# Dunni3/keypoint-diffusion

Measured on AMD Instinct MI355X. Metric: denoising steps/sec, higher is better.
Workload: dtype f32; 1 GPU; egnn_all_atom dynamics (6 EGNN layers, hidden 256, update_kp_feat; fixed receptor encoder), batch of 64 synthetic 300-atom pockets / 25-atom ligands per GPU, T=500, seeded random-init weights, every step taken from the t=T ligand state; batch_per_gpu=64, n_rec=300, n_lig=25, parallelism=dp1

## Files before the change

keypoint-diffusion_amd/csrc/egnn.hip:

```cpp
#include <string.h>

#include <map>
#include <set>
#include <string>
#include <vector>

#include "egnn_kernels.h"
#include "egnn_wide.h"
#include "mfma_core.h"

using namespace kpd;

namespace {

struct LayerW {
    float *wp_e[4], *wx_e[4], *b_e[4], *wr_e[4], *watt[4];
    float *wp_c[4], *wx_c[4], *b_c[4], *wr_c[4], *w3[4];
    void *wh_e[4], *wh_c[4];
    void *chh_p[2][NSLOT];
    void *wh_a[2], *wh_b[2], *wh_2[2];
    float *wp_p[2][NSLOT], *wx_p[2][NSLOT], *b_p[2][NSLOT];
    float *ch_p[2][NSLOT], *wcol_p[2][NSLOT];
    float *wp_a[2], *wx_a[2], *wp_b[2], *wx_b[2], *b0[2], *wp_2[2], *wx_2[2], *b2[2], *ln_w[2], *ln_b[2];
};
// ... 57 lines not shown
    int cap_B = 0, cap_lig = 0, cap_kp = 0, cap_kk = 0, cap_ll = 0, cap_kl = 0, cap_maxlig = 0, cap_maxkp = 0;
    int tile_cap = 0, tiles_et_cap[4] = {0, 0, 0, 0};
    float *h[2], *x[2], *P[2];
    float *hn_main[4], *hn_cont[4], *xn_main[4], *xn_cont[4];
    int *bidx[2];
    float *z[2];
    int *meta, *ll_deg, *ll_off, *kl_off, *kl_pg;
    kpd_lig_graph lg;
    int kp_table = 1;
    int tab_rows = 0;
    bool last_table = false;
    int *rowmap = nullptr, *kp_ok = nullptr;
    float *tab_in = nullptr;
    int *tab_bidx = nullptr;
    float *hT = nullptr, *PT = nullptr;
    EgnnWide *wide = nullptr;
};

static kpd_status build_weight_arena(kpd_egnn *m) {
    const kpd_egnn_config &c = m->cfg;
    m->warena.poison_at = 2;
    m->L.assign(c.n_layers, LayerW());
    return carve(m->warena, ARENA_TAIL, [&](Carve &A) {
        for (int i = 0; i < c.n_layers; ++i) {
            LayerW &w = m->L[i];
            const std::string pre = "egnn.conv_layers." + std::to_string(i) + ".";
            for (int et = 0; et < m->n_et; ++et) {
                A(w.wp_e[et], WP_FLOATS); A(w.wx_e[et], HS); A(w.b_e[et], HS); A(w.wr_e[et], HS); A(w.watt[et], HS);
                A(w.wp_c[et], WP_FLOATS); A(w.wx_c[et], HS); A(w.b_c[et], HS); A(w.wr_c[et], HS); A(w.w3[et], HS);
                A.as<unsigned short>(w.wh_e[et], WH_HALVES); A.as<unsigned short>(w.wh_c[et], WH_HALVES);
// ... 393 lines not shown
        }
        for (int et = 0; et < 4; ++et) {
            W.rows(m->hn_main[et], n[kDstNt[et]], HS, HW);
            W.rows(m->hn_cont[et], tiles[et], HS, HW);
            W(m->xn_main[et], (size_t)n[kDstNt[et]] * 4);
            W(m->xn_cont[et], (size_t)tiles[et] * 4);
        }
        carve_lig_graph(W, m->meta, m->ll_deg, m->ll_off, m->kl_off, m->kl_pg, g, max_B, max_n_lig, max_n_kp);
        if (tab_rows > 0) {
            W(m->rowmap, max_n_kp);
            W(m->kp_ok, 1);
            W(m->tab_in, (size_t)tab_rows * rec_nf);
            W(m->tab_bidx, tab_rows);
            W(m->hT, (size_t)(tab_rows + TM) * HS);
            W.rows(m->PT, (size_t)(tab_rows + TM) * NSLOT, HS, HW);
        }
    }));
    m->tab_rows = tab_rows;
    m->last_table = false;
    if (tab_rows > 0) {
        std::vector<float> in((size_t)tab_rows * rec_nf, 0.0f);
        std::vector<int> gi(tab_rows);
        for (int r = 0; r < tab_rows; ++r) {
            in[(size_t)r * rec_nf + r % rec_nf] = 1.0f;
            gi[r] = r / rec_nf;
        }
        KPD_HIP(hipMemcpy(m->tab_in, in.data(), in.size() * 4, hipMemcpyHostToDevice));
        KPD_HIP(hipMemcpy(m->tab_bidx, gi.data(), gi.size() * 4, hipMemcpyHostToDevice));
    }
    for (int et = 0; et < 4; ++et) m->tiles_et_cap[et] = tiles[et];
// ... 26 lines not shown
    if (kp_tab)
        KPD_TRY(launch_node_graph_index(bt->kp_ptr, bt->B, bt->n_kp, m->bidx[NT_KP], st, nullptr, bt->kp_h, c.rec_nf, m->rowmap, m->kp_ok));
    else
        KPD_TRY(launch_node_graph_index(bt->kp_ptr, bt->B, bt->n_kp, m->bidx[NT_KP], st));
    const float *x_cur[2] = {bt->lig_x, bt->kp_x};
    KPD_TRY(launch_lig_graph(bt, c.ll_cutoff, c.ll_k, c.kl_cutoff, c.kl_k, &m->lg, m->ll_deg, m->ll_off, m->kl_off, m->kl_pg, st));
    const int tr = TM;
    const int active = c.update_kp_feat ? 0xF : 0x3;
    const bool prune = c.update_kp_feat && m->prune_last;
    const int active_last = prune ? 0x3 : active;
    KPD_TRY(launch_egnn_meta(m->lg.counts, bt->n_kk, active, active_last, bt->lig_ptr, bt->kp_ptr, m->lg.ll_per_graph,
                             bt->kk_rowptr, bt->B, m->kl_off, c.message_norm, c.update_kp_feat, m->meta, m->z[NT_LIG],
                             m->z[NT_KP], st, tr));
    KPD_TRY(launch_embed(bt->lig_h, bt->n_lig, c.atom_nf, m->le_W0, m->le_b0, 64, m->le_W1t, m->le_b1, t_dev,
                         m->bidx[NT_LIG], m->h[NT_LIG], 0, st));
    KPD_TRY(launch_embed(bt->kp_h, bt->n_kp, c.rec_nf, m->re_W0, m->re_b0, 2 * c.rec_nf, m->re_W1t, m->re_b1, t_dev,
                         m->bidx[NT_KP], m->h[NT_KP], m->rec_identity ? 1 : 0, st));
    if (kp_tab) {
        KPD_REQUIRE(n_tab <= m->tab_rows, KPD_ERR_CAPACITY, "internal: %d class rows, table of %d", n_tab, m->tab_rows);
        KPD_TRY(launch_embed(m->tab_in, n_tab, c.rec_nf, m->re_W0, m->re_b0, 2 * c.rec_nf, m->re_W1t, m->re_b1, t_dev, m->tab_bidx,
                             m->hT, 0, st));
    }

    const int e_kl_cap = bt->n_kp * (c.kl_k > 0 ? c.kl_k : std::min(bt->max_lig, 100));
    const int E_cap[4] = {std::max<int>((long)bt->n_lig * std::min(bt->max_lig - 1, c.ll_k > 0 ? c.ll_k : 200), 1), e_kl_cap, e_kl_cap,
                          bt->n_kk};
    int tile_cap = 0, tile_cap_last = 0;
    for (int et = 0; et < m->n_et; ++et) {
        tile_cap += cdiv(E_cap[et], tr);
        if ((active_last >> et) & 1) tile_cap_last += cdiv(E_cap[et], tr);
    }

    const int n[2] = {bt->n_lig, bt->n_kp};
    const int *esrc[4] = {m->lg.ll_src, m->lg.kl_src, m->lg.lk_src, bt->kk_src};
    const int *edst[4] = {m->lg.ll_dst, m->lg.kl_dst, m->lg.lk_dst, bt->kk_dst};
    const int *rowptr[4] = {m->lg.ll_rowptr, m->lg.kl_rowptr, m->lg.lk_rowptr, bt->kk_rowptr};
    const int n_layers = m->debug_layers >= 0 ? std::min(m->debug_layers, c.n_layers) : c.n_layers;

    auto slot_mask = [&](int etmask, int nt) {
        int mk = 0;
        for (int et = 0; et < 4; ++et)
            if ((etmask >> et) & 1) {
                if (kSrcNt[et] == nt) mk |= 3 << kSrcSlot[et];
                if (kDstNt[et] == nt) mk |= 3 << kDstSlot[et];
            }
        return mk;
    };
    auto layer_etmask = [&](int li) { return li == n_layers - 1 ? active_last : active; };
    for (int li = 0; li < n_layers; ++li) {
        const LayerW &L = m->L[li];
        {
            {
// ... 8 lines not shown
                        if (L.wp_p[nt][s] && ((mk >> s) & 1)) {
                            pa.wp[k] = L.wp_p[nt][s]; pa.wx[k] = L.wx_p[nt][s]; pa.bias[k] = L.b_p[nt][s]; pa.slot[k] = s;
                            pa.chain[k] = L.ch_p[nt][s]; pa.wcol[k] = L.wcol_p[nt][s]; pa.chain_h[k] = L.chh_p[nt][s];
                            ++k;
                        }
                    pp.n_slots[nt] = k;
                }
                pp.tiles0 = cdiv(n[0], TM);
                pp.gemm_mode = m->gemm_mode;
                if (kp_tab && li == 0) {
                    ProjPair pk = pp;
                    pk.n_slots[NT_LIG] = 0;
                    pk.skip_if = m->kp_ok;
                    ProjArgs &pa = pp.nt[NT_KP];
                    pa.h = m->hT; pa.n = n_tab; pa.P = m->PT;
                    KPD_TRY(launch_proj_chain(pp, st));
                    KPD_TRY(launch_proj_chain(pk, st));
                } else {
                    KPD_TRY(launch_proj_chain(pp, st));
                }
            }
        }
        EdgeArgs ea;
        memset(&ea, 0, sizeof(ea));
        const bool last = li == n_layers - 1;
        ea.meta = last ? m->meta + 16 : m->meta;
        ea.x[0] = x_cur[0]; ea.x[1] = x_cur[1]; ea.P[0] = m->P[0]; ea.P[1] = m->P[1];
        ea.use_tanh = c.use_tanh; ea.coords_range = c.coords_range;
        ea.tile_rows = tr;
        ea.gemm_mode = tr == TM ? m->gemm_mode : 0;
        for (int et = 0; et < 4; ++et) {
            ea.src[et] = esrc[et]; ea.dst[et] = edst[et];
            ea.src_nt[et] = kSrcNt[et]; ea.dst_nt[et] = kDstNt[et]; ea.src_slot[et] = kSrcSlot[et]; ea.dst_slot[et] = kDstSlot[et];
            ea.wr_e[et] = L.wr_e[et]; ea.wr_c[et] = L.wr_c[et];
// ... 28 lines not shown
            na.ln_inv_n = 1.0f / (float)(c.hidden_nf + 1); na.ln_pad = (float)(HID - c.hidden_nf);
            na.wh_a = L.wh_a[nt]; na.wh_b = L.wh_b[nt]; na.wh_2 = L.wh_2[nt];
            na.norm = c.norm;
            na.tile_shift = 6;
        };
        {
            NodeLayerPair lp;
            memset(&lp, 0, sizeof(lp));
            for (int nt = 0; nt < 2; ++nt) {
                NodeLayerArgs &na = lp.nt[nt];
                na.u.n = n[nt]; na.u.h = m->h[nt];
                if (nt < m->n_upd && !(nt == NT_KP && last && prune)) {
                    fill_update(na.u, nt);
                    na.u.x_in = x_cur[nt] == m->x[nt] ? nullptr : x_cur[nt];
                    na.do_update = 1;
                }
                if (!na.do_update && !na.do_proj) na.u.n = 0;
            }
            lp.tiles0 = cdiv(lp.nt[0].u.n, TN);
            lp.gemm_mode = m->gemm_mode;
            KPD_TRY(launch_node_layer(lp, st));
            for (int nt = 0; nt < 2; ++nt)
                if (lp.nt[nt].do_update) x_cur[nt] = m->x[nt];
        }
    }
    if (x_cur[NT_LIG] != m->x[NT_LIG]) KPD_HIP(hipMemcpyAsync(m->x[NT_LIG], bt->lig_x, (size_t)bt->n_lig * 12, hipMemcpyDeviceToDevice, st));
    if (x_cur[NT_KP] != m->x[NT_KP]) KPD_HIP(hipMemcpyAsync(m->x[NT_KP], bt->kp_x, (size_t)bt->n_kp * 12, hipMemcpyDeviceToDevice, st));
    KPD_TRY(launch_decode(m->h[NT_LIG], m->x[NT_LIG], bt->lig_x, bt->n_lig, c.atom_nf, 2 * c.atom_nf, m->de_W0, m->de_b0,
                          m->de_W1, m->de_b1, eps_h, eps_x, st));
    return KPD_OK;
}

extern "C" kpd_status kpd_egnn_debug_state(kpd_egnn *m, const char *what, float *out, int64_t n_floats, void *stream) {
    KPD_REQUIRE(m && what && out, KPD_ERR_INVALID, "null argument");
    hipStream_t st = static_cast<hipStream_t>(stream);
    if (m->wide) return wide_debug_state(m->wide, what, out, n_floats, st);
    const std::string w(what);
    const float *src = nullptr;
    if (w == "h_lig") src = m->h[0];
    else if (w == "h_kp") src = m->h[1];
// ... 5 lines not shown
             w[3] >= '0' && w[3] < '4') {
        const int et = w[3] - '0';
        src = w[0] == 'x' ? (w[2] == 'm' ? m->xn_main[et] : m->xn_cont[et]) : (w[2] == 'm' ? m->hn_main[et] : m->hn_cont[et]);
    }
    else if (w == "kp_table_ok") {
        KPD_REQUIRE(n_floats == 1, KPD_ERR_INVALID, "kp_table_ok is one value");
        if (!m->last_table) {
            KPD_HIP(hipMemsetAsync(out, 0, 4, st));
            return KPD_OK;
        }
        src = reinterpret_cast<const float *>(m->kp_ok);
    } else if (w.rfind("kp_table=", 0) == 0) {
        m->kp_table = atoi(w.c_str() + 9);
        return KPD_OK;
    }
    else if (w.rfind("layers=", 0) == 0) {
        m->debug_layers = atoi(w.c_str() + 7);
        return KPD_OK;
    } else if (w.rfind("prune=", 0) == 0) {
        m->prune_last = atoi(w.c_str() + 6);
        return KPD_OK;
    } else if (w.rfind("gemm=", 0) == 0) {
        const std::string v = w.substr(5);
        KPD_REQUIRE(v == "f32" || v == "f16x2", KPD_ERR_INVALID, "gemm mode must be f32 or f16x2");
        KPD_REQUIRE(v == "f32" || !m->f32_only, KPD_ERR_INVALID,
                    "gemm=f16x2: atom_nf = %d / rec_nf = %d (hidden_nf = %d) run the exact fp32 path only; the f16x2 mode covers atom_nf <= 32 "
                    "with rec_nf <= 128 or 256, or the identity keypoint encoder at hidden_nf 256", m->cfg.atom_nf, m->cfg.rec_nf, m->cfg.hidden_nf);
        KPD_REQUIRE(v == "f32" || !m->committed || m->f16_ok, KPD_ERR_WEIGHTS, "%s", F16_RANGE_ERROR);
        m->gemm_mode = v == "f16x2" ? 1 : 0;
        return KPD_OK;
// ... 67 lines not shown
```

keypoint-diffusion_amd/csrc/egnn_chain.hip:

```cpp
#include <algorithm>
#include <cstdlib>

#include "chain_core.h"
#include "egnn_kernels.h"

namespace kpd {

namespace {

constexpr int ENT = 16;
constexpr int ECH4 = ENT * 64;

__device__ __forceinline__ float reduce_q(float v) {
    v += __shfl_xor(v, 16);
    v += __shfl_xor(v, 32);
    return v;
}

}

struct ProjWs {
    ProjPair p;
    int blocks0;
    int bpc[2];
    int tpb;
};

constexpr int WS_TILE = 128;
constexpr int WS_W4 = 16 * 8 * 64;
constexpr int WS_LDS_BYTES = WS_W4 * 16 + (128 + 128 + HS) * 4;

__global__ __launch_bounds__(512, 1) void k_proj_ws(ProjWs qa) {
    extern __shared__ __attribute__((aligned(16))) float smem[];
    v4f *W = reinterpret_cast<v4f *>(smem);
    float *s_wcol = smem + WS_W4 * 4, *s_bias = s_wcol + 128, *s_wrow = s_bias + 128;
    const int tid = threadIdx.x, wave = tid >> 6, lane = tid & 63;
    if (qa.p.skip_if && *qa.p.skip_if) return;
    const int which = (int)blockIdx.x >= qa.blocks0 ? 1 : 0;
    const ProjArgs &a = qa.p.nt[which];
    const int local = blockIdx.x - (which ? qa.blocks0 : 0);
    const int combo = local / qa.bpc[which], chunk = local - combo * qa.bpc[which];
    const int s = combo >> 1, hf = combo & 1;
    const int tiles = (a.n + WS_TILE - 1) / WS_TILE;
    const int t0 = chunk * qa.tpb, t1 = min(tiles, t0 + qa.tpb);
    if (t0 >= t1) return;
    {
        const v4f *src = reinterpret_cast<const v4f *>(a.chain[s]);
#pragma unroll
        for (int j = 0; j < WS_W4 / 512; ++j) {
            const int i = tid + 512 * j, ks = i >> 9, rem = i & 511;
            W[i] = src[(size_t)ks * ECH4 + 8 * hf * 64 + rem];
        }
        const float *bias = a.bias[s];
        if (tid < 128) {
            s_wcol[tid] = a.wcol[s][128 * hf + tid];
            s_bias[tid] = bias ? bias[128 * hf + tid] : 0.0f;
        }
        for (int i = tid; i < HS; i += 512) s_wrow[i] = i <= 256 ? a.wx[s][i] : 0.0f;
    }
    __syncthreads();
    const int el = lane & 15, q = lane >> 4;
    const float bias256 = a.bias[s] ? a.bias[s][256] : 0.0f;
    auto load_x = [&](int t, v4f (&x)[ENT], float &x256) {
        const int row = min(t * WS_TILE + 16 * wave + el, a.n - 1);
        const float *hrow = a.h + (size_t)row * HS;
#pragma unroll
        for (int nt = 0; nt < ENT; ++nt) x[nt] = *reinterpret_cast<const v4f *>(hrow + 16 * nt + 4 * q);
        x256 = hrow[256];
    };
    auto store_tile = [&](const v4f (&acc)[8], int row, float out256) {
        if (row >= 0 && row < a.n) {
            float *orow = a.P + ((size_t)row * NSLOT + a.slot[s]) * HS + 128 * hf;
#pragma unroll
            for (int m = 0; m < 8; ++m) *reinterpret_cast<v4f *>(orow + 16 * m + 4 * q) = acc[m];
            if (hf == 0 && q == 0) orow[256] = out256;
        }
    };
    v4f x[ENT], xn[ENT], accp[8];
    float h256, h256n, out256p = 0.0f;
    int rowp = -1;
#pragma unroll
    for (int m = 0; m < 8; ++m) accp[m] = zero4();
    load_x(t0, xn, h256n);
#pragma unroll 1
    for (int t = t0; t < t1; ++t) {
#pragma unroll
        for (int nt = 0; nt < ENT; ++nt)
#pragma unroll
            for (int r = 0; r < 4; ++r) asm volatile("v_mov_b32 %0, %1" : "=v"(x[nt][r]) : "v"(xn[nt][r]));
        asm volatile("v_mov_b32 %0, %1" : "=v"(h256) : "v"(h256n));
        __builtin_amdgcn_sched_barrier(0);
        store_tile(accp, rowp, out256p);
        if (t + 1 < t1) load_x(t + 1, xn, h256n);
        v4f acc[8];
#pragma unroll
        for (int m = 0; m < 8; ++m)
            acc[m] = h256 * *reinterpret_cast<const v4f *>(s_wcol + 16 * m + 4 * q) + *reinterpret_cast<const v4f *>(s_bias + 16 * m + 4 * q);
        float part = 0.0f;
        if (hf == 0) {
#pragma unroll
            for (int nt = 0; nt < ENT; ++nt) {
                const v4f wv = *reinterpret_cast<const v4f *>(s_wrow + 16 * nt + 4 * q);
                part += x[nt][0] * wv[0] + x[nt][1] * wv[1] + x[nt][2] * wv[2] + x[nt][3] * wv[3];
            }
        }
        const v4f *wp = W + lane;
        v4f w[2][4];
#pragma unroll
// ... 1 lines not shown
#pragma unroll
        for (int b = 0; b < 32; ++b) {
            if (b + 1 < 32) {
#pragma unroll
                for (int m = 0; m < 4; ++m) w[(b + 1) & 1][m] = wp[(4 * (b + 1) + m) * 64];
            }
            __builtin_amdgcn_sched_barrier(0);
            const v4f xin = x[b >> 1];
            const int g = b & 1;
#pragma unroll
            for (int r = 0; r < 4; ++r)
#pragma unroll
                for (int m = 0; m < 4; ++m) acc[4 * g + m] = mfma16(w[b & 1][m][r], xin[r], acc[4 * g + m]);
            __builtin_amdgcn_sched_barrier(0);
        }
        const int row = t * WS_TILE + 16 * wave + el;
        const float out256 = hf == 0 ? reduce_q(part) + bias256 + h256 * s_wrow[256] : 0.0f;
#pragma unroll
        for (int m = 0; m < 8; ++m) accp[m] = acc[m];
        rowp = row;
        out256p = out256;
    }
    store_tile(accp, rowp, out256p);
}

__global__ __launch_bounds__(512, 1) void k_proj_ws_h(ProjWs qa) {
    extern __shared__ __attribute__((aligned(16))) float smem[];
    f32x4 *W = reinterpret_cast<f32x4 *>(smem);
    float *s_wcol = smem + WS_W4 * 4, *s_bias = s_wcol + 128, *s_wrow = s_bias + 128;
    const int tid = threadIdx.x, wave = tid >> 6, lane = tid & 63;
    const int which = (int)blockIdx.x >= qa.blocks0 ? 1 : 0;
// ... 93 lines not shown
            acc[m0] = __builtin_amdgcn_mfma_f32_16x16x32_f16(as_h8(wb[1]), as_h8(xh[kb]), acc[m0], 0, 0, 0);
            acc[m0 + 1] = __builtin_amdgcn_mfma_f32_16x16x32_f16(as_h8(wb[3]), as_h8(xh[kb]), acc[m0 + 1], 0, 0, 0);
            acc[m0] = __builtin_amdgcn_mfma_f32_16x16x32_f16(as_h8(wb[0]), as_h8(xl[kb]), acc[m0], 0, 0, 0);
            acc[m0 + 1] = __builtin_amdgcn_mfma_f32_16x16x32_f16(as_h8(wb[2]), as_h8(xl[kb]), acc[m0 + 1], 0, 0, 0);
            acc[m0] = __builtin_amdgcn_mfma_f32_16x16x32_f16(as_h8(wb[0]), as_h8(xh[kb]), acc[m0], 0, 0, 0);
            acc[m0 + 1] = __builtin_amdgcn_mfma_f32_16x16x32_f16(as_h8(wb[2]), as_h8(xh[kb]), acc[m0 + 1], 0, 0, 0);
            __builtin_amdgcn_sched_barrier(0);
        }
#pragma unroll
        for (int m = 0; m < 8; ++m) accp[m] = H_UNSCALE * acc[m];
        rowp = row;
    }
    store_tile(accp, rowp);
}

kpd_status launch_proj_chain(const ProjPair &p, hipStream_t st) {
    const int slots = std::max(p.n_slots[0], p.n_slots[1]);
    if (poison_level() >= 1) KPD_TRY(poison_lds(st));
    if (slots == 0) return KPD_OK;
    for (int nt = 0; nt < 2; ++nt)
        for (int s = 0; s < p.n_slots[nt]; ++s)
            KPD_REQUIRE(p.nt[nt].chain[s] && p.nt[nt].wcol[s], KPD_ERR_STATE, "projection slot %d not packed", s);
    KPD_TRY(ensure_dynamic_lds(reinterpret_cast<const void *>(k_proj_ws), WS_LDS_BYTES));
    const int target = cu_count();
    ProjWs q;
    q.p = p;
    int units = 0, tl[2];
    for (int nt = 0; nt < 2; ++nt) {
        tl[nt] = p.n_slots[nt] ? cdiv(p.nt[nt].n, WS_TILE) : 0;
        units += 2 * p.n_slots[nt] * tl[nt];
    }
    if (units == 0) return KPD_OK;
    int blocks[2];
    for (q.tpb = std::max(1, cdiv(units, target));; ++q.tpb) {
        for (int nt = 0; nt < 2; ++nt) {
            q.bpc[nt] = std::max(1, cdiv(tl[nt], q.tpb));
            blocks[nt] = tl[nt] ? 2 * p.n_slots[nt] * q.bpc[nt] : 0;
        }
        if (blocks[0] + blocks[1] <= target || q.tpb >= std::max(tl[0], tl[1])) break;
    }
    q.blocks0 = blocks[0];
    if (p.gemm_mode == 1) {
        KPD_REQUIRE(!p.skip_if, KPD_ERR_INVALID, "projection launch: skip_if is served by the exact mode only");
        for (int nt = 0; nt < 2; ++nt)
            for (int s = 0; s < p.n_slots[nt]; ++s)
                KPD_REQUIRE(p.nt[nt].chain_h[s], KPD_ERR_STATE, "projection slot %d has no f16 planes (f16x2 mode)", s);
        KPD_TRY(ensure_dynamic_lds(reinterpret_cast<const void *>(k_proj_ws_h), WS_LDS_BYTES));
        hipLaunchKernelGGL(k_proj_ws_h, dim3(blocks[0] + blocks[1]), dim3(512), WS_LDS_BYTES, st, q);
        KPD_LAUNCH_CHECK();
        return KPD_OK;
    }
    hipLaunchKernelGGL(k_proj_ws, dim3(blocks[0] + blocks[1]), dim3(512), WS_LDS_BYTES, st, q);
    KPD_LAUNCH_CHECK();
    return KPD_OK;
}

}
```

keypoint-diffusion_amd/csrc/egnn_kernels.h:

```cpp
#pragma once
#include "engine.h"

namespace kpd {

constexpr int NSLOT = 8;
constexpr int ATT_BIAS_AT = 260;
constexpr int BIAS_K = 260;
constexpr int ET_LL = 0, ET_KL = 1, ET_LK = 2, ET_KK = 3;
constexpr int NT_LIG = 0, NT_KP = 1;

constexpr int EDGE_LDS_BYTES = TM * SA * 4 + (TM * 2 + TM + 3 * TM + TM + 3 * TM + 4 * HS + 8 + TM) * 4;
constexpr int EDGE_H_LDS_BYTES = 64 * 280 * 2 * 2 + (TM * 2 + TM + 3 * TM + TM + 3 * TM + 2 * HS + 8) * 4 + 2 * 2 * 272 * 2;

struct ProjArgs {
    const float *h;
    int n;
    float *P;
    const float *wp[NSLOT];
    const float *wx[NSLOT];
    const float *bias[NSLOT];
    int slot[NSLOT];
    const float *chain[NSLOT];
    const float *wcol[NSLOT];
    const void *chain_h[NSLOT];
// ... 86 lines not shown
    float *x;
    const float *x_in;
    const int *bidx;
    const float *z;
    int n_in;
    const int *rowptr[2];
    const float *hn_main[2], *hn_cont[2];
    const float *xn_main[2], *xn_cont[2];
    const float *wp_a, *wx_a, *wp_b, *wx_b, *b0;
    const float *wp_2, *wx_2, *b2;
    const void *wh_a, *wh_b, *wh_2;
    const float *ln_w, *ln_b;
    int norm;
    float ln_inv_n, ln_pad;
    int tile_shift;
};

struct NodeLayerArgs {
    NodeArgs u;
    int do_update, do_proj;
    float *P;
    int n_slots;
    const float *wp[NSLOT], *wx[NSLOT], *bias[NSLOT];
    int slot[NSLOT];
};

struct NodeLayerPair {
    NodeLayerArgs nt[2];
    int tiles0;
    int gemm_mode;
};

constexpr int TN = 32;
constexpr int NODE_LAYER_LDS_BYTES = TN * SA * 4 + 3 * TN * 4 + 3 * HS * 4;
constexpr int NODE_H_TILE_FLOATS = 2 * TN * 280 / 2;
constexpr int NODE_H_LDS_BYTES = NODE_H_TILE_FLOATS * 4 + 3 * TN * 4;


kpd_status egnn_kernels_init();
kpd_status launch_node_graph_index(const int *ptr, int B, int n, int *bidx, hipStream_t st, int *set_ok = nullptr,
                                   const float *kp_h = nullptr, int fin = 0, int *rowmap = nullptr, int *ok = nullptr);
kpd_status launch_egnn_meta(const int *counts, int e_kk, int active_mask, int active_last, const int *lig_ptr, const int *kp_ptr,
                            const int *ll_per_graph, const int *kk_rowptr, int B, const int *kl_off, float message_norm,
                            int update_kp, int *meta, float *z_lig, float *z_kp, hipStream_t st, int tile_rows = TM);
kpd_status launch_embed(const float *in, int n, int fin, const float *W0, const float *b0, int hid, const float *W1t,
                        const float *b1, const float *t, const int *bidx, float *out, int identity, hipStream_t st);
kpd_status launch_decode(const float *h, const float *x, const float *x0, int n, int atom_nf, int hid, const float *W0,
                         const float *b0, const float *W1, const float *b1, float *eps_h, float *eps_x, hipStream_t st);
kpd_status launch_egnn_edge(const EdgeArgs &a, int tile_cap, hipStream_t st);
kpd_status launch_egnn_edge_train(const EdgeTrainArgs &a, int tile_cap, hipStream_t st);
struct EdgePiecesSumArgs {
    const float *hn_main[4], *hn_cont[4], *xn_main[4], *xn_cont[4];
    const int *rowptr[4];
    int live[4], dst_nt[4];
    const float *zinv[2];
    int n[2];
    float *hn[2], *xn[2];
};
kpd_status launch_edge_pieces_sum(const EdgePiecesSumArgs &a, hipStream_t st);
kpd_status launch_edge_train_pack(const EdgePackTab &t, hipStream_t st);
kpd_status launch_egnn_edge_bwd(const EdgeBwdArgs &a, int tile_cap, hipStream_t st);
struct EdgePiecesBatch {
    struct One {
        const float *m1, *c1, *m2, *c2;
        const int *rowptr;
        int n;
        float *o1, *o2;
    } e[8];
    int ldo;
};
kpd_status launch_edge_pieces_set(const EdgePiecesBatch &b, int count, hipStream_t st);
kpd_status launch_proj_chain(const ProjPair &p, hipStream_t st);
kpd_status launch_node_layer(const NodeLayerPair &p, hipStream_t st);

}
```

keypoint-diffusion_amd/csrc/egnn_kernels.hip:

```cpp
#include <stdlib.h>

#include <algorithm>

#include "egnn_kernels.h"
#include "mfma_core.h"

namespace kpd {

__device__ __forceinline__ void kp_classify_row(const float *__restrict__ kp_h, int v, int graph, int fin, int *__restrict__ rowmap,
                                                int *__restrict__ ok) {
    const unsigned *row = reinterpret_cast<const unsigned *>(kp_h) + (size_t)v * fin;
    int ones = 0, other = 0, c = 0;
    for (int k = 0; k < fin; ++k) {
        const unsigned u = row[k];
        if (u == 0x3f800000u) { ++ones; c = k; }
        else if (u != 0u) other = 1;
    }
    rowmap[v] = graph * fin + c;
    if (ones != 1 || other) *ok = 0;
}

__global__ void k_node_graph_index(const int *__restrict__ ptr, int B, int n, int *__restrict__ bidx, int *__restrict__ set_ok,
                                   const float *__restrict__ kp_h, int fin, int *__restrict__ rowmap, int *__restrict__ ok) {
    const int i = blockIdx.x * blockDim.x + threadIdx.x;
// ... 33 lines not shown
            z_lig[b] = (float)(ll_per_graph[b] + e_kl) / (float)nl + 1.0f;
            z_kp[b] = update_kp ? (float)(e_kl + e_kk_b) / (float)nk + 1.0f : 1.0f;
        } else {
            z_lig[b] = message_norm;
            z_kp[b] = message_norm;
        }
    }
}

constexpr int EMB_NODES = 8;
template <int HMAX>
__global__ __launch_bounds__(256) void k_embed(const float *__restrict__ in, int n, int fin,
                                               const float *__restrict__ W0, const float *__restrict__ b0, int hid,
                                               const float *__restrict__ W1t, const float *__restrict__ b1,
                                               const float *__restrict__ t, const int *__restrict__ bidx,
                                               float *__restrict__ out, int identity) {
    __shared__ float s_in[EMB_NODES][256];
    __shared__ float s_hid[EMB_NODES][HMAX];
    const int node0 = blockIdx.x * EMB_NODES, tid = threadIdx.x;
    for (int i = tid; i < EMB_NODES * fin; i += 256) {
        const int j = i / fin, k = i - j * fin;
        s_in[j][k] = node0 + j < n ? in[(size_t)(node0 + j) * fin + k] : 0.0f;
    }
    __syncthreads();
    if (!identity) {
        for (int u = tid; u < hid; u += 256) {
            float a[EMB_NODES];
#pragma unroll
            for (int j = 0; j < EMB_NODES; ++j) a[j] = b0[u];
            for (int k = 0; k < fin; ++k) {
                const float w = W0[(size_t)u * fin + k];
// ... 1430 lines not shown
__global__ __launch_bounds__(512) __attribute__((amdgpu_waves_per_eu(6, 6))) void k_node_update8(NodeLayerPair p) {
    extern __shared__ __attribute__((aligned(16))) float smem[];
    float *A = smem;
    float *s_z = smem + TN * SA;
    float *s_mean = s_z + TN;
    float *s_rstd = s_mean + TN;
    float *s_wx = s_rstd + TN;
    const int tid = threadIdx.x, wave = __builtin_amdgcn_readfirstlane(tid >> 6), lane = tid & 63;
    const int which = blockIdx.x >= p.tiles0 ? 1 : 0;
    const NodeLayerArgs &L = p.nt[which];
    const NodeArgs &a = L.u;
    const int node0 = (blockIdx.x - (which ? p.tiles0 : 0)) * TN;
    constexpr int RPW = TN / 8;
    constexpr int TPR = 512 / TN;

    auto load_h = [&]() {
        f32x4 val[RPW], val2[RPW];
#pragma unroll
        for (int rr = 0; rr < RPW; ++rr) {
            const f32x4 *src = reinterpret_cast<const f32x4 *>(a.h + (size_t)(node0 + wave * RPW + rr) * HS);
            val[rr] = src[lane];
            val2[rr] = src[64 + (lane & 1)];
        }
#pragma unroll
        for (int rr = 0; rr < RPW; ++rr) {
            const int r = wave * RPW + rr;
            *reinterpret_cast<f32x4 *>(A + r * SA + 4 * lane) = val[rr];
            if (lane < 2) *reinterpret_cast<f32x4 *>(A + r * SA + 256 + 4 * lane) = val2[rr];
        }
    };
    const int two = a.n_in > 1 ? 1 : 0;
    const int *__restrict__ rp0 = a.rowptr[0], *__restrict__ rp1 = a.rowptr[two];

    f32x16 acc;
    {
// ... 18 lines not shown
                    for (int t = (lo1 >> a.tile_shift) + 1; t <= ((hi1 - 1) >> a.tile_shift); ++t) {
                        const float *q = a.xn_cont[two] + (size_t)t * 4;
                        sx += q[0]; sy += q[1]; sz += q[2];
                    }
                }
                float *xv = a.x + (size_t)v * 3;
                const float *xi = (a.x_in ? a.x_in : a.x) + (size_t)v * 3;
                xv[0] = xi[0] + sx / z; xv[1] = xi[1] + sy / z; xv[2] = xi[2] + sz / z;
            }
            s_z[tid] = z;
        } else if (tid >= 512 - 3 * 66) {
            const int i = tid - (512 - 3 * 66), which = i / 66, j = i - which * 66;
            const float *row = which == 0 ? a.wx_a : which == 1 ? a.wx_b : a.wx_2;
            reinterpret_cast<f32x4 *>(s_wx + which * HS)[j] = reinterpret_cast<const f32x4 *>(row)[j];
        }
        load_h();
        lds_barrier();
#pragma unroll
        for (int i = 0; i < 16; ++i) acc[i] = 0.0f;
        gemm_rows32_t8<NG, SA>(A, a.wp_a, acc, wave, lane);
        float ex = row_dot_chunks<TPR>(A, s_wx, KP / 4, tid);
        lds_barrier();
        {
            constexpr int GB = 2;
#pragma unroll
            for (int r0 = 0; r0 < RPW; r0 += GB) {
                int lo0[GB], hi0[GB], lo1[GB], hi1[GB];
                f32x4 m0[GB], m1[GB];
                float t0[GB], t1[GB];
#pragma unroll
                for (int rr = 0; rr < GB; ++rr) {
                    const int v = min(node0 + wave * RPW + r0 + rr, a.n - 1);
                    lo0[rr] = rp0[v]; hi0[rr] = rp0[v + 1];
                    lo1[rr] = rp1[v]; hi1[rr] = two ? rp1[v + 1] : lo1[rr];
                    const f32x4 *p0 = reinterpret_cast<const f32x4 *>(a.hn_main[0] + (size_t)v * HS);
                    const f32x4 *p1 = reinterpret_cast<const f32x4 *>(a.hn_main[two] + (size_t)v * HS);
                    m0[rr] = p0[lane]; t0[rr] = reinterpret_cast<const float *>(p0)[256 + (lane & 7)];
// ... 48 lines not shown
        for (int i = 0; i < 16; ++i) acc[i] = 0.0f;
        gemm_rows32_t8<NG, SA>(A, a.wp_2, acc, wave, lane);
        ex = row_dot_chunks<TPR>(A, s_wx + 2 * HS, KP / 4, tid);
        lds_barrier();
        {
            const int col = 32 * wave + (lane & 31);
            const float bb = a.b2[col];
#pragma unroll
            for (int reg = 0; reg < 16; ++reg) A[acc_row32(reg, lane) * SA + col] = acc[reg] + bb;
        }
        if ((tid % TPR) == 0) A[(tid / TPR) * SA + 256] = ex + a.b2[256];
        lds_barrier();
#pragma unroll 4
        for (int rr = 0; rr < RPW; ++rr) {
            const int r = wave * RPW + rr;
            const f32x4 *src = reinterpret_cast<const f32x4 *>(a.h + (size_t)(node0 + r) * HS);
            *reinterpret_cast<f32x4 *>(A + r * SA + 4 * lane) += src[lane];
            if (lane == 0) A[r * SA + 256] += a.h[(size_t)(node0 + r) * HS + 256];
        }
        lds_barrier();
        if (a.norm) {
            const int row = tid / TPR, q = tid % TPR;
            const float *tr = A + row * SA + q;
            float sum = 0.0f;
            for (int i = 0; i < 256 / TPR; ++i) sum += tr[TPR * i];
            if (q == 0) sum += A[row * SA + 256];
#pragma unroll
            for (int o = 1; o < TPR; o <<= 1) sum += __shfl_xor(sum, o);
            const float mean = sum * a.ln_inv_n;
            float var = 0.0f;
            for (int i = 0; i < 256 / TPR; ++i) {
                const float dlt = tr[TPR * i] - mean;
                var = fmaf(dlt, dlt, var);
// ... 22 lines not shown
                val = (val - mean) * rstd * w + b;
                last = (last - mean) * rstd * a.ln_w[256] + a.ln_b[256];
            }
            if (v >= a.n) {
                val = f32x4{0.f, 0.f, 0.f, 0.f};
                last = 0.0f;
            }
            *reinterpret_cast<f32x4 *>(A + r * SA + 4 * lane) = val;
            const f32x4 t = {last, 0.f, 0.f, 0.f};
            if (lane == 0) *reinterpret_cast<f32x4 *>(A + r * SA + 256) = t;
            if (lane == 1) *reinterpret_cast<f32x4 *>(A + r * SA + 260) = f32x4{0.f, 0.f, 0.f, 0.f};
            if (v < a.n) {
                f32x4 *dst = reinterpret_cast<f32x4 *>(a.h + (size_t)v * HS);
                dst[lane] = val;
                if (lane == 0) dst[64] = t;
            }
        }
        lds_barrier();
    }
}


__global__ __launch_bounds__(512) __attribute__((amdgpu_waves_per_eu(4, 6))) void k_node_update8_h(NodeLayerPair p) {
    extern __shared__ __attribute__((aligned(16))) float smem[];
    float *A = smem;
    _Float16 *Ah = reinterpret_cast<_Float16 *>(smem);
    constexpr int PN = TN * SAH;
    float *s_z = smem + NODE_H_TILE_FLOATS;
    float *s_mean = s_z + TN;
    float *s_rstd = s_mean + TN;
    const int tid = threadIdx.x, wave = tid >> 6, lane = tid & 63;
    const int which = blockIdx.x >= p.tiles0 ? 1 : 0;
    const NodeLayerArgs &L = p.nt[which];
    const NodeArgs &a = L.u;
// ... 175 lines not shown
    hipLaunchKernelGGL(k_node_graph_index, dim3(cdiv(n, 256)), dim3(256), 0, st, ptr, B, n, bidx, set_ok, kp_h, fin, rowmap, ok);
    KPD_LAUNCH_CHECK();
    return KPD_OK;
}

kpd_status launch_egnn_meta(const int *counts, int e_kk, int active_mask, int active_last, const int *lig_ptr, const int *kp_ptr,
                            const int *ll_per_graph, const int *kk_rowptr, int B, const int *kl_off, float message_norm,
                            int update_kp, int *meta, float *z_lig, float *z_kp, hipStream_t st, int tile_rows) {
    hipLaunchKernelGGL(k_egnn_meta, dim3(cdiv(B, 256)), dim3(256), 0, st, counts, e_kk, active_mask, active_last, lig_ptr, kp_ptr,
                       ll_per_graph, kk_rowptr, B, kl_off, message_norm, update_kp, tile_rows, meta, z_lig, z_kp);
    KPD_LAUNCH_CHECK();
    return KPD_OK;
}

kpd_status launch_embed(const float *in, int n, int fin, const float *W0, const float *b0, int hid, const float *W1t,
                        const float *b1, const float *t, const int *bidx, float *out, int identity, hipStream_t st) {
    if (n == 0) return KPD_OK;
    KPD_REQUIRE(fin <= 256 && hid <= 512, KPD_ERR_INVALID, "embed: fin=%d hid=%d exceed 256 / 512", fin, hid);
    if (hid <= 256 || identity)
        hipLaunchKernelGGL(k_embed<256>, dim3(cdiv(n, EMB_NODES)), dim3(256), 0, st, in, n, fin, W0, b0, hid, W1t, b1, t, bidx,
                           out, identity);
    else
        hipLaunchKernelGGL(k_embed<512>, dim3(cdiv(n, EMB_NODES)), dim3(256), 0, st, in, n, fin, W0, b0, hid, W1t, b1, t, bidx,
                           out, identity);
    KPD_LAUNCH_CHECK();
    return KPD_OK;
}

kpd_status launch_decode(const float *h, const float *x, const float *x0, int n, int atom_nf, int hid, const float *W0,
                         const float *b0, const float *W1, const float *b1, float *eps_h, float *eps_x,
                         hipStream_t st) {
    if (n == 0) return KPD_OK;
    KPD_REQUIRE(hid <= 512 && atom_nf <= 256, KPD_ERR_INVALID, "decode: hid=%d atom_nf=%d exceed 512 / 256", hid, atom_nf);
    if (hid <= 64 && atom_nf <= 64)
        hipLaunchKernelGGL(k_decode<64>, dim3(n), dim3(64), 0, st, h, x, x0, n, atom_nf, hid, W0, b0, W1, b1, eps_h, eps_x);
    else
        hipLaunchKernelGGL(k_decode<512>, dim3(n), dim3(64), 0, st, h, x, x0, n, atom_nf, hid, W0, b0, W1, b1, eps_h, eps_x);
    KPD_LAUNCH_CHECK();
    return KPD_OK;
// ... 27 lines not shown
}

kpd_status launch_node_layer(const NodeLayerPair &p, hipStream_t st) {
    const int tiles = p.tiles0 + cdiv(p.nt[1].u.n, TN);
    if (tiles == 0) return KPD_OK;
    if (poison_level() >= 1) KPD_TRY(poison_lds(st));
    for (int nt = 0; nt < 2; ++nt)
        KPD_REQUIRE(p.nt[nt].u.n == 0 || (p.nt[nt].do_update && !p.nt[nt].do_proj), KPD_ERR_INVALID, "node launch: update-only node types expected");
    for (int nt = 0; nt < 2; ++nt) {
        const NodeArgs &u = p.nt[nt].u;
        if (u.n == 0) continue;
        KPD_REQUIRE(u.n_in >= 1 && u.n_in <= 2, KPD_ERR_INVALID, "node launch: node type %d has %d incoming edge types (1 or 2 expected)", nt, u.n_in);
        for (int i = 0; i < u.n_in; ++i)
            KPD_REQUIRE(u.rowptr[i] && u.hn_main[i] && u.hn_cont[i] && u.xn_main[i] && u.xn_cont[i], KPD_ERR_INVALID,
                        "node launch: segment arrays of incoming edge type %d of node type %d are missing", i, nt);
    }
    if (p.gemm_mode == 1) {
        for (int nt = 0; nt < 2; ++nt)
            if (p.nt[nt].u.n > 0)
                KPD_REQUIRE(p.nt[nt].u.wh_a && p.nt[nt].u.wh_b && p.nt[nt].u.wh_2, KPD_ERR_STATE, "node weights of type %d have no f16 planes", nt);
        KPD_TRY(ensure_dynamic_lds(reinterpret_cast<const void *>(k_node_update8_h), NODE_H_LDS_BYTES));
        hipLaunchKernelGGL(k_node_update8_h, dim3(tiles), dim3(512), NODE_H_LDS_BYTES, st, p);
        KPD_LAUNCH_CHECK();
        return KPD_OK;
    }
    KPD_TRY(ensure_dynamic_lds(reinterpret_cast<const void *>(k_node_update8), NODE_LAYER_LDS_BYTES));
    hipLaunchKernelGGL(k_node_update8, dim3(tiles), dim3(512), NODE_LAYER_LDS_BYTES, st, p);
    KPD_LAUNCH_CHECK();
    return KPD_OK;
}


kpd_status launch_egnn_edge_train(const EdgeTrainArgs &a, int tile_cap, hipStream_t st) {
    if (tile_cap == 0) return KPD_OK;
    KPD_TRY(ensure_dynamic_lds(reinterpret_cast<const void *>(k_egnn_edge_train), EDGE_LDS_BYTES));
    hipLaunchKernelGGL(k_egnn_edge_train, dim3(8 * cdiv(tile_cap, 8)), dim3(256), EDGE_LDS_BYTES, st, a);
    KPD_LAUNCH_CHECK();
    return KPD_OK;
}

kpd_status launch_edge_pieces_sum(const EdgePiecesSumArgs &a, hipStream_t st) {
    const int most = std::max(a.n[0], a.n[1]);
    if (most == 0) return KPD_OK;
    hipLaunchKernelGGL(k_edge_pieces_sum, dim3(cdiv(most, 4), 2), dim3(256), 0, st, a);
    KPD_LAUNCH_CHECK();
    return KPD_OK;
}
// ... 28 lines not shown
```

Before: 157.0 steps/s.

## Use receptor class table for first node layer and finer projection work units

When keypoint features come from a small set of one-hot classes, the first layer's keypoint node update now reads embedded features from the class table via a row map. It can also use a precomputed first GEMM (gT) computed once per class, and the per-keypoint embed kernel is skipped when the table applies. Separately, the projection chain kernel gains a 64-row work unit, chosen automatically when per-block tile counts are small, to spread work across more CUs. This adds indirection, extra table memory and a second kernel template.

After: 157.7 steps/s, median of 6. Within noise of the previous version (+0.4%).

```diff
diff --git a/keypoint-diffusion_amd/csrc/egnn.hip b/keypoint-diffusion_amd/csrc/egnn.hip
--- a/keypoint-diffusion_amd/csrc/egnn.hip
+++ b/keypoint-diffusion_amd/csrc/egnn.hip
@@ -95,6 +95,10 @@
     float *tab_in = nullptr;
     int *tab_bidx = nullptr;
     float *hT = nullptr, *PT = nullptr;
+    int kp_table_node = 2;
+    float *gT = nullptr;
+    int proj_unit = 0;
+    float proj_plan = 0.0f;
     EgnnWide *wide = nullptr;
 };
 
@@ -518,6 +522,7 @@
             W(m->tab_bidx, tab_rows);
             W(m->hT, (size_t)(tab_rows + TM) * HS);
             W.rows(m->PT, (size_t)(tab_rows + TM) * NSLOT, HS, HW);
+            W(m->gT, (size_t)(tab_rows + TM) * HS);
         }
     }));
     m->tab_rows = tab_rows;
@@ -574,12 +579,16 @@
                              m->z[NT_KP], st, tr));
     KPD_TRY(launch_embed(bt->lig_h, bt->n_lig, c.atom_nf, m->le_W0, m->le_b0, 64, m->le_W1t, m->le_b1, t_dev,
                          m->bidx[NT_LIG], m->h[NT_LIG], 0, st));
+    const int n_layers = m->debug_layers >= 0 ? std::min(m->debug_layers, c.n_layers) : c.n_layers;
+    const bool tab_node = kp_tab && m->kp_table_node > 0 && c.update_kp_feat && n_layers >= 1 && !(n_layers == 1 && prune);
     KPD_TRY(launch_embed(bt->kp_h, bt->n_kp, c.rec_nf, m->re_W0, m->re_b0, 2 * c.rec_nf, m->re_W1t, m->re_b1, t_dev,
-                         m->bidx[NT_KP], m->h[NT_KP], m->rec_identity ? 1 : 0, st));
+                         m->bidx[NT_KP], m->h[NT_KP], m->rec_identity ? 1 : 0, st, tab_node ? m->kp_ok : nullptr));
     if (kp_tab) {
         KPD_REQUIRE(n_tab <= m->tab_rows, KPD_ERR_CAPACITY, "internal: %d class rows, table of %d", n_tab, m->tab_rows);
         KPD_TRY(launch_embed(m->tab_in, n_tab, c.rec_nf, m->re_W0, m->re_b0, 2 * c.rec_nf, m->re_W1t, m->re_b1, t_dev, m->tab_bidx,
                              m->hT, 0, st));
+        if (tab_node && m->kp_table_node > 1)
+            KPD_TRY(launch_node_gemm1a(m->hT, n_tab, m->L[0].wp_a[NT_KP], m->L[0].wx_a[NT_KP], m->gT, st));
     }
 
     const int e_kl_cap = bt->n_kp * (c.kl_k > 0 ? c.kl_k : std::min(bt->max_lig, 100));
@@ -595,7 +604,14 @@
     const int *esrc[4] = {m->lg.ll_src, m->lg.kl_src, m->lg.lk_src, bt->kk_src};
     const int *edst[4] = {m->lg.ll_dst, m->lg.kl_dst, m->lg.lk_dst, bt->kk_dst};
     const int *rowptr[4] = {m->lg.ll_rowptr, m->lg.kl_rowptr, m->lg.lk_rowptr, bt->kk_rowptr};
-    const int n_layers = m->debug_layers >= 0 ? std::min(m->debug_layers, c.n_layers) : c.n_layers;
+    m->proj_plan = 0.0f;
+    int plan = 0;
+    auto proj = [&](const ProjPair &pp) {
+        int unit = 0;
+        KPD_TRY(launch_proj_chain(pp, st, m->proj_unit, &unit));
+        plan |= unit == 64 ? 1 : unit == 128 ? 2 : 0;
+        return KPD_OK;
+    };
 
     auto slot_mask = [&](int etmask, int nt) {
         int mk = 0;
@@ -634,10 +650,10 @@
                     pk.skip_if = m->kp_ok;
                     ProjArgs &pa = pp.nt[NT_KP];
                     pa.h = m->hT; pa.n = n_tab; pa.P = m->PT;
-                    KPD_TRY(launch_proj_chain(pp, st));
-                    KPD_TRY(launch_proj_chain(pk, st));
+                    KPD_TRY(proj(pp));
+                    KPD_TRY(proj(pk));
                 } else {
-                    KPD_TRY(launch_proj_chain(pp, st));
+                    KPD_TRY(proj(pp));
                 }
             }
         }
@@ -696,6 +712,10 @@
                     fill_update(na.u, nt);
                     na.u.x_in = x_cur[nt] == m->x[nt] ? nullptr : x_cur[nt];
                     na.do_update = 1;
+                    if (nt == NT_KP && li == 0 && tab_node) {
+                        na.u.h_tab = m->hT; na.u.h_map = m->rowmap; na.u.ok = m->kp_ok;
+                        na.u.g_tab = m->kp_table_node > 1 ? m->gT : nullptr;
+                    }
                 }
                 if (!na.do_update && !na.do_proj) na.u.n = 0;
             }
@@ -706,6 +726,7 @@
                 if (lp.nt[nt].do_update) x_cur[nt] = m->x[nt];
         }
     }
+    m->proj_plan = (float)plan;
     if (x_cur[NT_LIG] != m->x[NT_LIG]) KPD_HIP(hipMemcpyAsync(m->x[NT_LIG], bt->lig_x, (size_t)bt->n_lig * 12, hipMemcpyDeviceToDevice, st));
     if (x_cur[NT_KP] != m->x[NT_KP]) KPD_HIP(hipMemcpyAsync(m->x[NT_KP], bt->kp_x, (size_t)bt->n_kp * 12, hipMemcpyDeviceToDevice, st));
     KPD_TRY(launch_decode(m->h[NT_LIG], m->x[NT_LIG], bt->lig_x, bt->n_lig, c.atom_nf, 2 * c.atom_nf, m->de_W0, m->de_b0,
@@ -741,6 +762,21 @@
         m->kp_table = atoi(w.c_str() + 9);
         return KPD_OK;
     }
+    else if (w.rfind("kp_table_node=", 0) == 0) {
+        const int v = atoi(w.c_str() + 14);
+        KPD_REQUIRE(v >= 0 && v <= 2, KPD_ERR_INVALID, "kp_table_node must be 0, 1 or 2");
+        m->kp_table_node = v;
+        return KPD_OK;
+    } else if (w.rfind("proj_unit=", 0) == 0) {
+        const int v = atoi(w.c_str() + 10);
+        KPD_REQUIRE(v == 0 || v == 64 || v == 128, KPD_ERR_INVALID, "proj_unit must be 0, 64 or 128");
+        m->proj_unit = v;
+        return KPD_OK;
+    } else if (w == "proj_plan") {
+        KPD_REQUIRE(n_floats == 1, KPD_ERR_INVALID, "proj_plan is one value");
+        KPD_HIP(hipMemcpyAsync(out, &m->proj_plan, 4, hipMemcpyHostToDevice, st));
+        return KPD_OK;
+    }
     else if (w.rfind("layers=", 0) == 0) {
         m->debug_layers = atoi(w.c_str() + 7);
         return KPD_OK;
diff --git a/keypoint-diffusion_amd/csrc/egnn_chain.hip b/keypoint-diffusion_amd/csrc/egnn_chain.hip
--- a/keypoint-diffusion_amd/csrc/egnn_chain.hip
+++ b/keypoint-diffusion_amd/csrc/egnn_chain.hip
@@ -24,12 +24,14 @@
     int blocks0;
     int bpc[2];
     int tpb;
+    int upb[2];
 };
 
 constexpr int WS_TILE = 128;
 constexpr int WS_W4 = 16 * 8 * 64;
 constexpr int WS_LDS_BYTES = WS_W4 * 16 + (128 + 128 + HS) * 4;
 
+template <int UNIT>
 __global__ __launch_bounds__(512, 1) void k_proj_ws(ProjWs qa) {
     extern __shared__ __attribute__((aligned(16))) float smem[];
     v4f *W = reinterpret_cast<v4f *>(smem);
@@ -41,9 +43,13 @@
     const int local = blockIdx.x - (which ? qa.blocks0 : 0);
     const int combo = local / qa.bpc[which], chunk = local - combo * qa.bpc[which];
     const int s = combo >> 1, hf = combo & 1;
-    const int tiles = (a.n + WS_TILE - 1) / WS_TILE;
-    const int t0 = chunk * qa.tpb, t1 = min(tiles, t0 + qa.tpb);
+    const int tiles = (a.n + UNIT - 1) / UNIT;
+    const int per = UNIT == WS_TILE ? qa.tpb : qa.upb[which];
+    const int t0 = chunk * per, t1 = min(tiles, t0 + per);
     if (t0 >= t1) return;
+    const int base = UNIT == WS_TILE ? 0 : t0 * UNIT;
+    const int ta = UNIT == WS_TILE ? t0 : 0;
+    const int tb = UNIT == WS_TILE ? t1 : __builtin_amdgcn_readfirstlane((min(a.n, t1 * UNIT) - base - 16 * wave + WS_TILE - 1) / WS_TILE);
     {
         const v4f *src = reinterpret_cast<const v4f *>(a.chain[s]);
 #pragma unroll
@@ -59,10 +65,11 @@
         for (int i = tid; i < HS; i += 512) s_wrow[i] = i <= 256 ? a.wx[s][i] : 0.0f;
     }
     __syncthreads();
+    if (UNIT != WS_TILE && tb <= 0) return;
     const int el = lane & 15, q = lane >> 4;
     const float bias256 = a.bias[s] ? a.bias[s][256] : 0.0f;
     auto load_x = [&](int t, v4f (&x)[ENT], float &x256) {
-        const int row = min(t * WS_TILE + 16 * wave + el, a.n - 1);
+        const int row = min(base + t * WS_TILE + 16 * wave + el, a.n - 1);
         const float *hrow = a.h + (size_t)row * HS;
 #pragma unroll
         for (int nt = 0; nt < ENT; ++nt) x[nt] = *reinterpret_cast<const v4f *>(hrow + 16 * nt + 4 * q);
@@ -81,9 +88,9 @@
     int rowp = -1;
 #pragma unroll
     for (int m = 0; m < 8; ++m) accp[m] = zero4();
-    load_x(t0, xn, h256n);
+    load_x(ta, xn, h256n);
 #pragma unroll 1
-    for (int t = t0; t < t1; ++t) {
+    for (int t = ta; t < tb; ++t) {
 #pragma unroll
         for (int nt = 0; nt < ENT; ++nt)
 #pragma unroll
@@ -91,7 +98,7 @@
         asm volatile("v_mov_b32 %0, %1" : "=v"(h256) : "v"(h256n));
         __builtin_amdgcn_sched_barrier(0);
         store_tile(accp, rowp, out256p);
-        if (t + 1 < t1) load_x(t + 1, xn, h256n);
+        if (t + 1 < tb) load_x(t + 1, xn, h256n);
         v4f acc[8];
 #pragma unroll
         for (int m = 0; m < 8; ++m)
@@ -123,7 +130,7 @@
                 for (int m = 0; m < 4; ++m) acc[4 * g + m] = mfma16(w[b & 1][m][r], xin[r], acc[4 * g + m]);
             __builtin_amdgcn_sched_barrier(0);
         }
-        const int row = t * WS_TILE + 16 * wave + el;
+        const int row = base + t * WS_TILE + 16 * wave + el;
         const float out256 = hf == 0 ? reduce_q(part) + bias256 + h256 * s_wrow[256] : 0.0f;
 #pragma unroll
         for (int m = 0; m < 8; ++m) accp[m] = acc[m];
@@ -247,17 +254,22 @@
     store_tile(accp, rowp);
 }
 
-kpd_status launch_proj_chain(const ProjPair &p, hipStream_t st) {
+constexpr int WS_UNIT = 64;
+constexpr int WS_COARSE_TPB = 6;
+
+kpd_status launch_proj_chain(const ProjPair &p, hipStream_t st, int force_unit, int *unit_used) {
     const int slots = std::max(p.n_slots[0], p.n_slots[1]);
     if (poison_level() >= 1) KPD_TRY(poison_lds(st));
     if (slots == 0) return KPD_OK;
+    KPD_REQUIRE(force_unit == 0 || force_unit == WS_TILE || force_unit == WS_UNIT, KPD_ERR_INVALID, "projection launch: unit %d (0, 64 or 128)", force_unit);
     for (int nt = 0; nt < 2; ++nt)
         for (int s = 0; s < p.n_slots[nt]; ++s)
             KPD_REQUIRE(p.nt[nt].chain[s] && p.nt[nt].wcol[s], KPD_ERR_STATE, "projection slot %d not packed", s);
-    KPD_TRY(ensure_dynamic_lds(reinterpret_cast<const void *>(k_proj_ws), WS_LDS_BYTES));
+    KPD_TRY(ensure_dynamic_lds(reinterpret_cast<const void *>(k_proj_ws<WS_TILE>), WS_LDS_BYTES));
     const int target = cu_count();
     ProjWs q;
     q.p = p;
+    q.upb[0] = q.upb[1] = 0;
     int units = 0, tl[2];
     for (int nt = 0; nt < 2; ++nt) {
         tl[nt] = p.n_slots[nt] ? cdiv(p.nt[nt].n, WS_TILE) : 0;
@@ -281,9 +293,33 @@
         KPD_TRY(ensure_dynamic_lds(reinterpret_cast<const void *>(k_proj_ws_h), WS_LDS_BYTES));
         hipLaunchKernelGGL(k_proj_ws_h, dim3(blocks[0] + blocks[1]), dim3(512), WS_LDS_BYTES, st, q);
         KPD_LAUNCH_CHECK();
+        if (unit_used) *unit_used = WS_TILE;
         return KPD_OK;
     }
-    hipLaunchKernelGGL(k_proj_ws, dim3(blocks[0] + blocks[1]), dim3(512), WS_LDS_BYTES, st, q);
+    const bool fine = force_unit ? force_unit == WS_UNIT : q.tpb < WS_COARSE_TPB;
+    if (unit_used) *unit_used = fine ? WS_UNIT : WS_TILE;
+    if (!fine) {
+        hipLaunchKernelGGL(k_proj_ws<WS_TILE>, dim3(blocks[0] + blocks[1]), dim3(512), WS_LDS_BYTES, st, q);
+        KPD_LAUNCH_CHECK();
+        return KPD_OK;
+    }
+    int ul[2];
+    units = 0;
+    for (int nt = 0; nt < 2; ++nt) {
+        ul[nt] = p.n_slots[nt] ? cdiv(p.nt[nt].n, WS_UNIT) : 0;
+        units += 2 * p.n_slots[nt] * ul[nt];
+    }
+    for (int most = std::max(1, cdiv(units, target));; ++most) {
+        for (int nt = 0; nt < 2; ++nt) {
+            q.bpc[nt] = std::max(1, cdiv(ul[nt], most));
+            q.upb[nt] = std::max(1, cdiv(ul[nt], q.bpc[nt]));
+            blocks[nt] = ul[nt] ? 2 * p.n_slots[nt] * q.bpc[nt] : 0;
+        }
+        if (blocks[0] + blocks[1] <= target || most >= std::max(ul[0], ul[1])) break;
+    }
+    q.blocks0 = blocks[0];
+    KPD_TRY(ensure_dynamic_lds(reinterpret_cast<const void *>(k_proj_ws<WS_UNIT>), WS_LDS_BYTES));
+    hipLaunchKernelGGL(k_proj_ws<WS_UNIT>, dim3(blocks[0] + blocks[1]), dim3(512), WS_LDS_BYTES, st, q);
     KPD_LAUNCH_CHECK();
     return KPD_OK;
 }
diff --git a/keypoint-diffusion_amd/csrc/egnn_kernels.h b/keypoint-diffusion_amd/csrc/egnn_kernels.h
--- a/keypoint-diffusion_amd/csrc/egnn_kernels.h
+++ b/keypoint-diffusion_amd/csrc/egnn_kernels.h
@@ -124,6 +124,8 @@
     int norm;
     float ln_inv_n, ln_pad;
     int tile_shift;
+    const float *h_tab, *g_tab;
+    const int *h_map, *ok;
 };
 
 struct NodeLayerArgs {
@@ -154,7 +156,8 @@
                             const int *ll_per_graph, const int *kk_rowptr, int B, const int *kl_off, float message_norm,
                             int update_kp, int *meta, float *z_lig, float *z_kp, hipStream_t st, int tile_rows = TM);
 kpd_status launch_embed(const float *in, int n, int fin, const float *W0, const float *b0, int hid, const float *W1t,
-                        const float *b1, const float *t, const int *bidx, float *out, int identity, hipStream_t st);
+                        const float *b1, const float *t, const int *bidx, float *out, int identity, hipStream_t st,
+                        const int *skip_if = nullptr);
 kpd_status launch_decode(const float *h, const float *x, const float *x0, int n, int atom_nf, int hid, const float *W0,
                          const float *b0, const float *W1, const float *b1, float *eps_h, float *eps_x, hipStream_t st);
 kpd_status launch_egnn_edge(const EdgeArgs &a, int tile_cap, hipStream_t st);
@@ -180,7 +183,8 @@
     int ldo;
 };
 kpd_status launch_edge_pieces_set(const EdgePiecesBatch &b, int count, hipStream_t st);
-kpd_status launch_proj_chain(const ProjPair &p, hipStream_t st);
+kpd_status launch_proj_chain(const ProjPair &p, hipStream_t st, int force_unit = 0, int *unit_used = nullptr);
 kpd_status launch_node_layer(const NodeLayerPair &p, hipStream_t st);
+kpd_status launch_node_gemm1a(const float *hT, int n, const float *wp_a, const float *wx_a, float *G, hipStream_t st);
 
 }
diff --git a/keypoint-diffusion_amd/csrc/egnn_kernels.hip b/keypoint-diffusion_amd/csrc/egnn_kernels.hip
--- a/keypoint-diffusion_amd/csrc/egnn_kernels.hip
+++ b/keypoint-diffusion_amd/csrc/egnn_kernels.hip
@@ -71,7 +71,8 @@
                                                const float *__restrict__ W0, const float *__restrict__ b0, int hid,
                                                const float *__restrict__ W1t, const float *__restrict__ b1,
                                                const float *__restrict__ t, const int *__restrict__ bidx,
-                                               float *__restrict__ out, int identity) {
+                                               float *__restrict__ out, int identity, const int *__restrict__ skip_if) {
+    if (skip_if && *skip_if) return;
     __shared__ float s_in[EMB_NODES][256];
     __shared__ float s_hid[EMB_NODES][HMAX];
     const int node0 = blockIdx.x * EMB_NODES, tid = threadIdx.x;
@@ -1532,11 +1533,17 @@
     constexpr int RPW = TN / 8;
     constexpr int TPR = 512 / TN;
 
+    const bool tab = a.h_tab != nullptr && *a.ok != 0;
+    const bool pre = tab && a.g_tab != nullptr;
+    auto h_row = [&](int r) -> const float * {
+        const int v = node0 + r;
+        return tab ? a.h_tab + (size_t)a.h_map[min(v, a.n - 1)] * HS : a.h + (size_t)v * HS;
+    };
     auto load_h = [&]() {
         f32x4 val[RPW], val2[RPW];
 #pragma unroll
         for (int rr = 0; rr < RPW; ++rr) {
-            const f32x4 *src = reinterpret_cast<const f32x4 *>(a.h + (size_t)(node0 + wave * RPW + rr) * HS);
+            const f32x4 *src = reinterpret_cast<const f32x4 *>(h_row(wave * RPW + rr));
             val[rr] = src[lane];
             val2[rr] = src[64 + (lane & 1)];
         }
@@ -1585,13 +1592,25 @@
             const float *row = which == 0 ? a.wx_a : which == 1 ? a.wx_b : a.wx_2;
             reinterpret_cast<f32x4 *>(s_wx + which * HS)[j] = reinterpret_cast<const f32x4 *>(row)[j];
         }
-        load_h();
-        lds_barrier();
-#pragma unroll
-        for (int i = 0; i < 16; ++i) acc[i] = 0.0f;
-        gemm_rows32_t8<NG, SA>(A, a.wp_a, acc, wave, lane);
-        float ex = row_dot_chunks<TPR>(A, s_wx, KP / 4, tid);
-        lds_barrier();
+        float ex;
+        if (pre) {
+            const int col = 32 * wave + (lane & 31);
+#pragma unroll
+            for (int reg = 0; reg < 16; ++reg) {
+                const int v = min(node0 + acc_row32(reg, lane), a.n - 1);
+                acc[reg] = a.g_tab[(size_t)a.h_map[v] * HS + col];
+            }
+            ex = a.g_tab[(size_t)a.h_map[min(node0 + tid / TPR, a.n - 1)] * HS + 256];
+            lds_barrier();
+        } else {
+            load_h();
+            lds_barrier();
+#pragma unroll
+            for (int i = 0; i < 16; ++i) acc[i] = 0.0f;
+            gemm_rows32_t8<NG, SA>(A, a.wp_a, acc, wave, lane);
+            ex = row_dot_chunks<TPR>(A, s_wx, KP / 4, tid);
+            lds_barrier();
+        }
         {
             constexpr int GB = 2;
 #pragma unroll
@@ -1670,9 +1689,9 @@
 #pragma unroll 4
         for (int rr = 0; rr < RPW; ++rr) {
             const int r = wave * RPW + rr;
-            const f32x4 *src = reinterpret_cast<const f32x4 *>(a.h + (size_t)(node0 + r) * HS);
+            const f32x4 *src = reinterpret_cast<const f32x4 *>(h_row(r));
             *reinterpret_cast<f32x4 *>(A + r * SA + 4 * lane) += src[lane];
-            if (lane == 0) A[r * SA + 256] += a.h[(size_t)(node0 + r) * HS + 256];
+            if (lane == 0) A[r * SA + 256] += reinterpret_cast<const float *>(src)[256];
         }
         lds_barrier();
         if (a.norm) {
@@ -1725,10 +1744,50 @@
                 f32x4 *dst = reinterpret_cast<f32x4 *>(a.h + (size_t)v * HS);
                 dst[lane] = val;
                 if (lane == 0) dst[64] = t;
+                if (lane == 1) dst[65] = f32x4{0.f, 0.f, 0.f, 0.f};
             }
         }
         lds_barrier();
     }
+}
+
+
+__global__ __launch_bounds__(512) void k_node_gemm1a(const float *__restrict__ hT, int n, const float *__restrict__ wp_a,
+                                                     const float *__restrict__ wx_a, float *__restrict__ G) {
+    __shared__ __attribute__((aligned(16))) float A[TN * SA];
+    __shared__ __attribute__((aligned(16))) float s_wx[HS];
+    const int tid = threadIdx.x, wave = __builtin_amdgcn_readfirstlane(tid >> 6), lane = tid & 63;
+    const int node0 = blockIdx.x * TN;
+    constexpr int RPW = TN / 8, TPR = 512 / TN;
+    if (tid < 66) reinterpret_cast<f32x4 *>(s_wx)[tid] = reinterpret_cast<const f32x4 *>(wx_a)[tid];
+    {
+        f32x4 val[RPW], val2[RPW];
+#pragma unroll
+        for (int rr = 0; rr < RPW; ++rr) {
+            const f32x4 *src = reinterpret_cast<const f32x4 *>(hT + (size_t)(node0 + wave * RPW + rr) * HS);
+            val[rr] = src[lane];
+            val2[rr] = src[64 + (lane & 1)];
+        }
+#pragma unroll
+        for (int rr = 0; rr < RPW; ++rr) {
+            const int r = wave * RPW + rr;
+            *reinterpret_cast<f32x4 *>(A + r * SA + 4 * lane) = val[rr];
+            if (lane < 2) *reinterpret_cast<f32x4 *>(A + r * SA + 256 + 4 * lane) = val2[rr];
+        }
+    }
+    lds_barrier();
+    f32x16 acc;
+#pragma unroll
+    for (int i = 0; i < 16; ++i) acc[i] = 0.0f;
+    gemm_rows32_t8<NG, SA>(A, wp_a, acc, wave, lane);
+    const float ex = row_dot_chunks<TPR>(A, s_wx, KP / 4, tid);
+    const int col = 32 * wave + (lane & 31);
+#pragma unroll
+    for (int reg = 0; reg < 16; ++reg) {
+        const int v = node0 + acc_row32(reg, lane);
+        if (v < n) G[(size_t)v * HS + col] = acc[reg];
+    }
+    if ((tid % TPR) == 0 && node0 + tid / TPR < n) G[(size_t)(node0 + tid / TPR) * HS + 256] = ex;
 }
 
 
@@ -1934,15 +1993,15 @@
 }
 
 kpd_status launch_embed(const float *in, int n, int fin, const float *W0, const float *b0, int hid, const float *W1t,
-                        const float *b1, const float *t, const int *bidx, float *out, int identity, hipStream_t st) {
+                        const float *b1, const float *t, const int *bidx, float *out, int identity, hipStream_t st, const int *skip_if) {
     if (n == 0) return KPD_OK;
     KPD_REQUIRE(fin <= 256 && hid <= 512, KPD_ERR_INVALID, "embed: fin=%d hid=%d exceed 256 / 512", fin, hid);
     if (hid <= 256 || identity)
         hipLaunchKernelGGL(k_embed<256>, dim3(cdiv(n, EMB_NODES)), dim3(256), 0, st, in, n, fin, W0, b0, hid, W1t, b1, t, bidx,
-                           out, identity);
+                           out, identity, skip_if);
     else
         hipLaunchKernelGGL(k_embed<512>, dim3(cdiv(n, EMB_NODES)), dim3(256), 0, st, in, n, fin, W0, b0, hid, W1t, b1, t, bidx,
-                           out, identity);
+                           out, identity, skip_if);
     KPD_LAUNCH_CHECK();
     return KPD_OK;
 }
@@ -2000,6 +2059,8 @@
         for (int i = 0; i < u.n_in; ++i)
             KPD_REQUIRE(u.rowptr[i] && u.hn_main[i] && u.hn_cont[i] && u.xn_main[i] && u.xn_cont[i], KPD_ERR_INVALID,
                         "node launch: segment arrays of incoming edge type %d of node type %d are missing", i, nt);
+        KPD_REQUIRE(!u.h_tab ? !u.g_tab : (u.h_map && u.ok && p.gemm_mode == 0), KPD_ERR_INVALID,
+                    "node launch: class table of node type %d without its row map or flag, or outside the exact mode", nt);
     }
     if (p.gemm_mode == 1) {
         for (int nt = 0; nt < 2; ++nt)
@@ -2017,6 +2078,14 @@
 }
 
 
+kpd_status launch_node_gemm1a(const float *hT, int n, const float *wp_a, const float *wx_a, float *G, hipStream_t st) {
+    if (n == 0) return KPD_OK;
+    KPD_REQUIRE(hT && wp_a && wx_a && G, KPD_ERR_INVALID, "node GEMM 1a: null argument");
+    hipLaunchKernelGGL(k_node_gemm1a, dim3(cdiv(n, TN)), dim3(512), 0, st, hT, n, wp_a, wx_a, G);
+    KPD_LAUNCH_CHECK();
+    return KPD_OK;
+}
+
 kpd_status launch_egnn_edge_train(const EdgeTrainArgs &a, int tile_cap, hipStream_t st) {
     if (tile_cap == 0) return KPD_OK;
     KPD_TRY(ensure_dynamic_lds(reinterpret_cast<const void *>(k_egnn_edge_train), EDGE_LDS_BYTES));
```
